# AITRICS/Medical_Tri_Modal_Pilot

Measured on AMD Instinct MI355X. Metric: tri-modal training samples/s (fwd+bwd+AdamW step, per-GPU batch 64), higher is better.
Workload: dtype bf16; 1 GPU; BASELINE configs[1]: vslt_img_txt tri_mbt_vsltcls, 6 layers, d_model 256, batch 64/GPU, TIE-len 1000 (N_v=1005), 224x224 CXR, 128-tok text, dropout 0.1, mbt-only-vslt 1, imgtxt-time 1; global_batch=64, parallelism=dp1

## Files before the change

include/mtmp.h:

```cpp
#ifndef MTMP_H
#define MTMP_H
#include <stdint.h>
#ifdef __cplusplus
extern "C" {
#endif

#define MTMP_F32 0
#define MTMP_BF16 1

int mtmp_abi_version(void);
const char* mtmp_last_error(void);

int mtmp_attn_fwd(int dtype, const void* q, const void* k, const void* v, void* o, const void* res, void* o_res,
                  float* lse, const int32_t* kv_len, const float* key_norms, int B, int N, int H, int ld_qkv, int ld_o,
                  float scale, void* stream);
int mtmp_attn_fwd_grouped(int dtype, int n, const void* const* q, const void* const* k, const void* const* v, void* const* o,
                          const void* const* res, void* const* o_res, float* const* lse, const int32_t* const* kv_len,
                          const int32_t* const* row_start, const float* const* key_norms, const int* N, const int* ld_qkv,
                          const int* ld_o, int B, int H, float scale, void* stream);
int mtmp_attn_bwd_grouped(int dtype, int n, const void* const* q, const void* const* k, const void* const* v,
                          const void* const* o, const void* const* d_o, const float* const* lse, const int32_t* const* kv_len,
                          const int32_t* const* row_start, void* const* dq, void* const* dk, void* const* dv,
                          float* const* delta_ws, const int* N, const int* ld_qkv, const int* ld_o, const int* ld_do,
                          const int* ld_dqkv, int B, int H, float scale, void* stream);
// ... 125 lines not shown
                             void* stream);
int mtmp_ln_gemm_signs_grouped(int dtype, int n, const void* const* x, const float* const* gamma, const float* const* beta,
                               const void* const* w, const float* const* bias, void* const* y, void* const* xn, float* const* stats,
                               void* const* signs, const int* M, int N, const int* ldx, float eps, float drop_p,
                               const unsigned* seeds, const unsigned* seed_dev, const int32_t* const* rows_live, void* stream);
int mtmp_gemm_nt_grouped(int dtype, int n, const void* const* a, const void* const* w, const float* const* bias,
                         const void* const* res, void* const* y, const int* M, int N, int K, const int* lda, const int* ldy,
                         const int* ldr, int act, float drop_p, const unsigned* seeds, const unsigned* seed_dev,
                         const int32_t* const* rows_live, void* stream);
int mtmp_gemm_nt_signs_drop_grouped(int dtype, int n, const void* const* a, const void* const* w, void* const* y, const int* M, int N,
                                    const int* lda, const void* const* signs, float gate_scale, float drop_p, const unsigned* seeds,
                                    const unsigned* seed_dev, void* const* a_out, const int32_t* const* rows_live, void* stream);
int mtmp_gemm_lnbwd_grouped(int dtype, int n, const void* const* dy, const void* const* wt, const void* const* z, const int* ldz,
                            const float* const* stats, const float* const* gamma, const void* const* d_res, const int* ldr,
                            void* const* dz, float* const* ws, const int* M, int K, const int* ldy, float eps,
                            const int32_t* const* rows_live, void* stream);
int mtmp_gemm_tn_group_plan(int n, const int* M, int N, int K, int* splits_out);
int mtmp_gemm_tn_grouped(int dtype, int n, const void* const* dy, const void* const* x, float* const* ws, const int* M, int N, int K,
                         const int* ldy, const int* ldx, const int* splits, const int32_t* const* rows_live, void* stream);

int mtmp_gemm_tn_slab_rows(int dtype, int M, int N, int K);
int mtmp_gemm_lnbwd_slab_rows(int M);
int mtmp_reduce_batch(const float* const* slab, const int* rows, const long long* cols, float* const* out_a, const long long* split,
                      float* const* out_b, int n, void* stream);

int mtmp_stream_input_slab_rows(int rows);
int mtmp_stream_input_bwd_partials(int dtype, const void* dz, const void* x, const float* cls, const float* gamma, const float* stats,
                                   void* dx, float* ws, int B, int N, int nb, float p, unsigned seed, const unsigned* seed_dev,
                                   const int32_t* row_start, const int32_t* kv_len, void* stream);
int mtmp_stream_input_bwd_grouped(int dtype, int n, const void* const* dz, const void* const* x, const float* const* cls,
                                  const float* const* gamma, const float* const* stats, void* const* dx, float* ws, const int* B,
                                  const int* N, const int* nb, const float* p, const unsigned* seed, const unsigned* seed_dev,
                                  const int32_t* const* row_start, const int32_t* const* kv_len, const void* const* add,
                                  const int* add_L, void* stream);
int mtmp_stream_input_fwd_add(int dtype, const void* x, const float* cls, const float* gamma, const float* beta, const float* pe,
                              const float* bott, void* out, float* stats, int B, int N, int nb, float eps, float p, unsigned seed,
                              const unsigned* seed_dev, const int32_t* row_start, const int32_t* kv_len, const void* add,
                              int add_L, void* stream);
int mtmp_token_sums(int dtype, int n, const void* const* dx, void* const* out, const int* rows, const int* L, void* stream);
int mtmp_tie_bwd_slab_rows(int n);
int mtmp_tie_time_embed_bwd_partials(int dtype, const float* events, int n, const float* time_events, int n_time, int n_time_a,
                                     const float* params, const void* d_out, const void* d_time_a, const void* d_time_b, float* ws,
                                     void* stream);
int mtmp_reduce_scatter(const float* const* src, const int* rows, const long long* ld, const long long* cols, float* const* out, int n,
                        void* stream);

int mtmp_publish_scalar(const float* value, unsigned* pair, void* stream);

int mtmp_copy_batch(const void* const* src, void* const* dst, const long long* bytes, const int* round16, int n, void* stream);

int mtmp_transpose_batch(int elem_bytes, const void* const* src, void* const* dst, const int* rows, const int* cols, int n,
                         void* stream);

int mtmp_stream_lengths(const long long* len_v, const long long* len_i, const long long* len_t, int* out, int B, int n_bott,
                        int txt_idx, void* stream);
int mtmp_image_slots(const long long* pattern, int present_below, int32_t* out, int B, int hw0, void* stream);
int mtmp_swin_stem_fwd_live(int dtype, const float* img, const float* w, const float* bias, const float* ln_w, const float* ln_b,
                            void* out, int n_img, int H, int W, const int32_t* order, const int32_t* rows_live, void* stream);
int mtmp_layernorm_rows_live(int dtype, const void* x, const float* w, const float* b, void* y, long long rows, int C, float eps,
                             int merge, int H, int W, const int32_t* rows_live, void* stream);
int mtmp_swin_ln_linear_live(int dtype, const void* x, const float* ln_w, const float* ln_b, const void* w, const float* bias,
                             void* y, long long M, int C, int N, float eps, const int32_t* rows_live, void* stream);
int mtmp_swin_mlp_live(int dtype, const void* x, const float* ln_w, const float* ln_b, const void* w1, const float* b1,
                       const void* w2, const float* b2, const float* row_scale, int rows_per_scale, void* y, long long M, int C,
                       float eps, const int32_t* rows_live, void* stream);
int mtmp_swin_window_attn_live(int dtype, const void* qkv, const void* table, void* out, int n_img, int H, int W, int C, int heads,
                               int shift, float scale, const int32_t* rows_live, void* stream);

int mtmp_layernorm_rows_bwd_slab_rows(long long rows, int C);
int mtmp_layernorm_rows_bwd(int dtype, const void* x, const float* w, const void* dy, void* dx, float* slab, long long rows, int C,
                            float eps, void* stream);
int mtmp_gelu_fwd(int dtype, const void* x, void* y, long long n, void* stream);
int mtmp_gelu_bwd(int dtype, const void* x, const void* dy, void* dx, long long n, void* stream);
int mtmp_swin_window_attn_bwd(int dtype, const void* qkv, const void* table, const void* dout, void* dqkv, float* dtab, int n_img,
                              int H, int W, int C, int heads, int shift, float scale, void* stream);

int mtmp_swin_attn_block(int dtype, const void* x, const float* ln_w, const float* ln_b, float eps, const void* wqkv,
                         const float* bqkv, const void* table, const void* wproj, const float* bproj, const float* row_scale,
                         void* out, int n_img, int H, int W, int C, int heads, int shift, float scale, const int32_t* rows_live,
                         void* stream);
int mtmp_gemm_nt_live(int dtype, const void* a, const void* w, const float* bias, const void* res, void* y, int M, int N, int K,
                      int lda, int ldy, int ldr, int act, float drop_p, unsigned seed, const unsigned* seed_dev, const void* gate,
                      float gate_scale, const float* row_scale, int rows_per_scale, const int32_t* rows_live, void* stream);

int mtmp_row_starts(const int32_t* kv_len, int32_t* out, int B, int n_max, void* stream);

#ifdef __cplusplus
}
#endif
#endif
```

medical_tri_modal_pilot_amd/_lib.py:

```python
import ctypes
import os
from ctypes import c_char_p, c_float, c_int, c_longlong, c_uint, c_void_p

_HERE = os.path.dirname(os.path.abspath(__file__))
LIB_PATH = os.environ.get("MTMP_LIB", os.path.join(_HERE, "libmtmp_hip.so"))

F32, BF16 = 0, 1

SIGNATURES = {
    "mtmp_abi_version": (c_int, []),
    "mtmp_last_error": (c_char_p, []),
    "mtmp_attn_fwd": (c_int, [c_int] + [c_void_p] * 9 + [c_int] * 5 + [c_float, c_void_p]),
    "mtmp_attn_cls_fwd": (c_int, [c_int] + [c_void_p] * 3 + [c_int, c_void_p, c_int] + [c_void_p] * 5 + [c_int] * 4 + [c_float, c_void_p]),
    "mtmp_attn_cls_bwd": (c_int, [c_int] + [c_void_p] * 3 + [c_int] + [c_void_p] * 8 + [c_int] * 5 + [c_float, c_void_p]),
    "mtmp_attn_fwd_grouped": (c_int, [c_int, c_int] + [c_void_p] * 13 + [c_int, c_int, c_float, c_void_p]),
    "mtmp_attn_bwd_grouped": (c_int, [c_int, c_int] + [c_void_p] * 17 + [c_int, c_int, c_float, c_void_p]),
    "mtmp_key_norms_floats": (c_longlong, [c_longlong, c_int]),
    "mtmp_key_norms": (c_int, [c_int, c_void_p, c_void_p, c_longlong, c_int, c_int, c_void_p]),
    "mtmp_attn_bwd": (c_int, [c_int] + [c_void_p] * 11 + [c_int] * 7 + [c_float, c_void_p]),
    "mtmp_ln_gemm": (c_int, [c_int] + [c_void_p] * 8 + [c_int] * 4 + [c_float, c_int, c_float, c_uint, c_void_p, c_void_p]),
    "mtmp_ln_gemm_qkv": (c_int, [c_int] + [c_void_p] * 9 + [c_int, c_int, c_float, c_void_p]),
    "mtmp_gemm_nt": (c_int, [c_int] + [c_void_p] * 5 + [c_int] * 7 + [c_float, c_uint, c_void_p, c_void_p, c_float, c_void_p, c_int,
                             c_void_p]),
    "mtmp_gemm_nt_live": (c_int, [c_int] + [c_void_p] * 5 + [c_int] * 7 + [c_float, c_uint, c_void_p, c_void_p, c_float, c_void_p, c_int,
                             c_void_p, c_void_p]),
    "mtmp_sign_bits_bytes": (c_longlong, [c_int, c_int]),
    "mtmp_ln_gemm_signs": (c_int, [c_int] + [c_void_p] * 8 + [c_int] * 4 + [c_float, c_float, c_uint, c_void_p, c_void_p, c_void_p]),
    "mtmp_gemm_nt_signs": (c_int, [c_int] + [c_void_p] * 3 + [c_int] * 4 + [c_void_p, c_float, c_void_p]),
    "mtmp_gemm_nt_signs_drop": (c_int, [c_int] + [c_void_p] * 3 + [c_int] * 4 + [c_void_p, c_float, c_float, c_uint, c_void_p,
                                                                                   c_void_p, c_void_p]),
    "mtmp_ln_gemm_qkv_grouped": (c_int, [c_int, c_int] + [c_void_p] * 11 + [c_float, c_void_p, c_void_p]),
    "mtmp_ln_gemm_signs_grouped": (c_int, [c_int, c_int] + [c_void_p] * 10 + [c_int, c_void_p, c_float, c_float, c_void_p, c_void_p,
                                                                                   c_void_p, c_void_p]),
    "mtmp_gemm_nt_grouped": (c_int, [c_int, c_int] + [c_void_p] * 6 + [c_int, c_int] + [c_void_p] * 3 + [c_int, c_float, c_void_p,
                                                                                                       c_void_p, c_void_p, c_void_p]),
    "mtmp_gemm_nt_signs_drop_grouped": (c_int, [c_int, c_int] + [c_void_p] * 4 + [c_int, c_void_p, c_void_p, c_float, c_float,
                                                                                  c_void_p, c_void_p, c_void_p, c_void_p, c_void_p]),
    "mtmp_gemm_lnbwd_grouped": (c_int, [c_int, c_int] + [c_void_p] * 11 + [c_int, c_void_p, c_float, c_void_p, c_void_p]),
    "mtmp_gemm_tn_group_plan": (c_int, [c_int, c_void_p, c_int, c_int, c_void_p]),
    "mtmp_gemm_tn_grouped": (c_int, [c_int, c_int] + [c_void_p] * 4 + [c_int, c_int] + [c_void_p] * 4 + [c_void_p]),
    "mtmp_gemm_tn_slab_rows": (c_int, [c_int] * 4),
    "mtmp_gemm_lnbwd_slab_rows": (c_int, [c_int]),
    "mtmp_reduce_batch": (c_int, [c_void_p] * 6 + [c_int, c_void_p]),
    "mtmp_reduce_scatter": (c_int, [c_void_p] * 5 + [c_int, c_void_p]),
    "mtmp_stream_input_slab_rows": (c_int, [c_int]),
    "mtmp_stream_input_bwd_partials": (c_int, [c_int] + [c_void_p] * 7 + [c_int] * 3 + [c_float, c_uint, c_void_p, c_void_p, c_void_p, c_void_p]),
    "mtmp_stream_input_bwd_grouped": (c_int, [c_int, c_int] + [c_void_p] * 18),
    "mtmp_stream_input_fwd_add": (c_int, [c_int] + [c_void_p] * 8 + [c_int] * 3 + [c_float, c_float, c_uint, c_void_p, c_void_p, c_void_p, c_void_p, c_int, c_void_p]),
    "mtmp_token_sums": (c_int, [c_int, c_int] + [c_void_p] * 5),
    "mtmp_tie_bwd_slab_rows": (c_int, [c_int]),
    "mtmp_tie_time_embed_bwd_partials": (c_int, [c_int, c_void_p, c_int, c_void_p, c_int, c_int] + [c_void_p] * 6),
    "mtmp_publish_scalar": (c_int, [c_void_p, c_void_p, c_void_p]),
    "mtmp_copy_batch": (c_int, [c_void_p] * 4 + [c_int, c_void_p]),
    "mtmp_stream_lengths": (c_int, [c_void_p] * 4 + [c_int] * 3 + [c_void_p]),
    "mtmp_row_starts": (c_int, [c_void_p, c_void_p, c_int, c_int, c_void_p]),
    "mtmp_image_slots": (c_int, [c_void_p, c_int, c_void_p, c_int, c_int, c_void_p]),
    "mtmp_transpose_batch": (c_int, [c_int, c_void_p, c_void_p, c_void_p, c_void_p, c_int, c_void_p]),
    "mtmp_layernorm_rows": (c_int, [c_int] + [c_void_p] * 4 + [c_longlong, c_int, c_float, c_int, c_int, c_int, c_void_p]),
    "mtmp_layernorm_rows_live": (c_int, [c_int] + [c_void_p] * 4 + [c_longlong, c_int, c_float, c_int, c_int, c_int, c_void_p, c_void_p]),
    "mtmp_swin_window_attn": (c_int, [c_int] + [c_void_p] * 3 + [c_int] * 6 + [c_float, c_void_p]),
    "mtmp_swin_window_attn_live": (c_int, [c_int] + [c_void_p] * 3 + [c_int] * 6 + [c_float, c_void_p, c_void_p]),
    "mtmp_layernorm_rows_bwd_slab_rows": (c_int, [c_longlong, c_int]),
    "mtmp_layernorm_rows_bwd": (c_int, [c_int] + [c_void_p] * 5 + [c_longlong, c_int, c_float, c_void_p]),
    "mtmp_gelu_fwd": (c_int, [c_int, c_void_p, c_void_p, c_longlong, c_void_p]),
    "mtmp_gelu_bwd": (c_int, [c_int, c_void_p, c_void_p, c_void_p, c_longlong, c_void_p]),
    "mtmp_swin_window_attn_bwd": (c_int, [c_int] + [c_void_p] * 5 + [c_int] * 6 + [c_float, c_void_p]),
    "mtmp_gemm_tn_ws_floats": (c_longlong, [c_int, c_int, c_int]),
    "mtmp_gemm_tn": (c_int, [c_int] + [c_void_p] * 5 + [c_int] * 5 + [c_void_p]),
    "mtmp_gemm_tn_live": (c_int, [c_int] + [c_void_p] * 5 + [c_int] * 5 + [c_void_p, c_void_p]),
    "mtmp_ln_bwd_ws_floats": (c_int, [c_int]),
    "mtmp_ln_bwd": (c_int, [c_int, c_void_p, c_int, c_void_p, c_void_p, c_void_p, c_void_p, c_int, c_void_p,
                            c_void_p, c_void_p, c_int, c_float, c_void_p]),
    "mtmp_gemm_lnbwd_ws_floats": (c_int, [c_int]),
    "mtmp_gemm_lnbwd": (c_int, [c_int, c_void_p, c_void_p, c_void_p, c_int, c_void_p, c_void_p, c_void_p, c_int, c_void_p,
                                c_void_p, c_void_p, c_int, c_int, c_int, c_float, c_void_p]),
    "mtmp_tie_embed_fwd": (c_int, [c_int] + [c_void_p] * 4 + [c_int, c_void_p]),
    "mtmp_tie_bwd_ws_floats": (c_int, [c_int]),
    "mtmp_tie_embed_bwd": (c_int, [c_int] + [c_void_p] * 5 + [c_int, c_void_p]),
    "mtmp_time_embed_fwd": (c_int, [c_int] + [c_void_p] * 4 + [c_int, c_void_p]),
    "mtmp_time_embed_bwd": (c_int, [c_int] + [c_void_p] * 5 + [c_int, c_void_p]),
    "mtmp_tie_embed_packed_fwd": (c_int, [c_int, c_void_p, c_void_p, c_int, c_int, c_void_p, c_void_p, c_void_p, c_void_p]),
    "mtmp_tie_embed_packed_bwd": (c_int, [c_int, c_void_p, c_void_p, c_int, c_int, c_void_p, c_void_p, c_void_p, c_void_p, c_void_p]),
    "mtmp_stream_input_ws_floats": (c_int, [c_int]),
    "mtmp_stream_input_fwd": (c_int, [c_int] + [c_void_p] * 8 + [c_int] * 3 + [c_float, c_float, c_uint, c_void_p, c_void_p, c_void_p, c_void_p]),
    "mtmp_stream_input_bwd": (c_int, [c_int] + [c_void_p] * 8 + [c_int] * 3 + [c_float, c_uint, c_void_p, c_void_p, c_void_p, c_void_p]),
    "mtmp_head_ws_floats": (c_int, [c_int]),
    "mtmp_head_fwd": (c_int, [c_void_p] * 6 + [c_int, c_float, c_float, c_float, c_int, c_void_p]),
    "mtmp_head_bwd": (c_int, [c_void_p] * 12 + [c_int, c_float, c_int, c_void_p]),
    "mtmp_head_fwd_t": (c_int, [c_int] + [c_void_p] * 6 + [c_int, c_float, c_float, c_float, c_int, c_void_p, c_void_p]),
    "mtmp_head_bwd_scatter": (c_int, [c_int] + [c_void_p] * 9 + [c_int, c_float, c_int, c_void_p]),
    "mtmp_bce_logits_mean": (c_int, [c_void_p] * 4 + [c_int, c_void_p]),
    "mtmp_timestamp": (c_int, [c_void_p, c_void_p]),
    "mtmp_swin_ln_linear": (c_int, [c_int] + [c_void_p] * 6 + [c_longlong, c_int, c_int, c_float, c_void_p]),
    "mtmp_swin_ln_linear_live": (c_int, [c_int] + [c_void_p] * 6 + [c_longlong, c_int, c_int, c_float, c_void_p, c_void_p]),
    "mtmp_swin_mlp": (c_int, [c_int] + [c_void_p] * 8 + [c_int, c_void_p, c_longlong, c_int, c_float, c_void_p]),
    "mtmp_swin_mlp_live": (c_int, [c_int] + [c_void_p] * 8 + [c_int, c_void_p, c_longlong, c_int, c_float, c_void_p, c_void_p]),
    "mtmp_swin_attn_block": (c_int, [c_int] + [c_void_p] * 3 + [c_float] + [c_void_p] * 7 + [c_int] * 6 + [c_float, c_void_p, c_void_p]),
    "mtmp_swin_stem_fwd": (c_int, [c_int] + [c_void_p] * 6 + [c_int] * 3 + [c_void_p]),
    "mtmp_swin_stem_fwd_live": (c_int, [c_int] + [c_void_p] * 6 + [c_int] * 3 + [c_void_p, c_void_p, c_void_p]),
    "mtmp_adamw_step": (c_int, [c_void_p] * 5 + [c_longlong] + [c_float] * 5 + [c_int, c_float, c_void_p]),
    "mtmp_bottleneck_exchange_fwd": (c_int, [c_int] + [c_void_p] * 3 + [c_int] * 4 + [c_void_p, c_int, c_void_p, c_void_p, c_void_p, c_void_p]),
    "mtmp_bottleneck_exchange_bwd": (c_int, [c_int] + [c_void_p] * 3 + [c_int] * 4 + [c_void_p, c_int, c_void_p, c_void_p, c_void_p, c_void_p]),
    "mtmp_dropout_bwd": (c_int, [c_int, c_void_p, c_void_p, c_longlong, c_uint, c_void_p, c_float, c_void_p]),
}

_lib = None


# ... 24 lines not shown
```

medical_tri_modal_pilot_amd/csrc/gemm.hip:

```cpp
#include "common.hip.h"
#include <type_traits>
template <int N> using template_int = std::integral_constant<int, N>;

namespace {

constexpr int BM = 128, BN = 128, BK = 64, LDW = BK + 8;

template <typename T> struct GemmArgs {
    const T* a; const T* w; const float* bias; const T* res; T* y;
    const float* gamma; const float* beta; T* xn; float* stats;
    int M, N, K, lda, ldy, ldr;
    float eps;
    float drop_p;
    unsigned seed;
    const unsigned* seed_dev;
    const T* gate;
    float gate_scale;
    int act;
    const float* row_scale;
    int rows_per_scale;
    unsigned short* signs = nullptr;
    float* knorm = nullptr;
    const int* m_live = nullptr;
};
// ... 1149 lines not shown
        g.seg[i] = segs[i < n ? i : 0];
        g.first[i] = total;
        if (i < n) total += blocks_of(segs[i]);
    }
    g.first[GRP_MAX] = total;
    return g;
}

int launch_ln_gemm_dma(int n, const GemmArgs<bf16>* segs, int relu, int gate, hipStream_t st) {
    using P = PanelDma;
    const GemmArgs<bf16>& a = segs[0];
    const bool drop = a.drop_p > 0.f, signs = !gate && relu && a.signs;
    for (int i = 1; i < n; ++i)
        if (segs[i].N != a.N || (segs[i].drop_p > 0.f) != drop || !segs[i].signs != !a.signs || !segs[i].knorm != !a.knorm ||
            !segs[i].gamma != !a.gamma) {
            mtmp_set_error("mtmp_ln_gemm (grouped): the streams of one launch must agree in N, dropout, sign bits and key norms");
            return MTMP_ERR_ARG;
        }
    const void* fs[7] = {(const void*)ln_gemm_dma_kernel<false, false, false, false>, (const void*)ln_gemm_dma_kernel<false, true, false, false>,
                         (const void*)ln_gemm_dma_kernel<true, false, false, false>, (const void*)ln_gemm_dma_kernel<true, true, false, false>,
                         (const void*)ln_gemm_dma_kernel<true, false, false, true>, (const void*)ln_gemm_dma_kernel<true, true, false, true>,
                         (const void*)ln_gemm_dma_kernel<false, false, true, false>};
    const bool knorm = a.knorm != nullptr;
    const int which = gate ? 6 : signs ? 4 + (drop ? 1 : 0) : (relu ? 2 : 0) + (drop ? 1 : 0);
    const void* fk = (const void*)ln_gemm_dma_kernel<false, false, false, false, true>;
    if (hipFuncSetAttribute(knorm ? fk : fs[which], hipFuncAttributeMaxDynamicSharedMemorySize, (int)P::lds_bytes) != hipSuccess) {
        mtmp_set_error("mtmp_ln_gemm: cannot raise dynamic LDS to %zu", P::lds_bytes);
        return MTMP_ERR_LAUNCH;
    }
    int mtiles;
    const Grouped<GemmArgs<bf16>> g = make_group(n, segs, [](const GemmArgs<bf16>& x) { return (x.M + BM - 1) / BM; }, mtiles);
    const int npanels = a.N / P::NP;
    int nsplit = 512 / mtiles;
    nsplit = nsplit < 1 ? 1 : (nsplit > npanels ? npanels : nsplit);
    const int need = (npanels + P::MAXP - 1) / P::MAXP;
    if (nsplit < need) nsplit = need;
    dim3 grid(mtiles, nsplit);
    if (knorm) {
        hipLaunchKernelGGL((ln_gemm_dma_kernel<false, false, false, false, true>), grid, dim3(256), P::lds_bytes, st, g);
        MTMP_CHECK_LAUNCH("mtmp_ln_gemm_qkv");
        return MTMP_OK;
    }
    switch (which) {
    case 0: hipLaunchKernelGGL((ln_gemm_dma_kernel<false, false, false, false>), grid, dim3(256), P::lds_bytes, st, g); break;
    case 1: hipLaunchKernelGGL((ln_gemm_dma_kernel<false, true, false, false>), grid, dim3(256), P::lds_bytes, st, g); break;
    case 2: hipLaunchKernelGGL((ln_gemm_dma_kernel<true, false, false, false>), grid, dim3(256), P::lds_bytes, st, g); break;
    case 3: hipLaunchKernelGGL((ln_gemm_dma_kernel<true, true, false, false>), grid, dim3(256), P::lds_bytes, st, g); break;
    case 4: hipLaunchKernelGGL((ln_gemm_dma_kernel<true, false, false, true>), grid, dim3(256), P::lds_bytes, st, g); break;
    case 5: hipLaunchKernelGGL((ln_gemm_dma_kernel<true, true, false, true>), grid, dim3(256), P::lds_bytes, st, g); break;
    default: hipLaunchKernelGGL((ln_gemm_dma_kernel<false, false, true, false>), grid, dim3(256), P::lds_bytes, st, g); break;
    }
    MTMP_CHECK_LAUNCH("mtmp_ln_gemm");
    return MTMP_OK;
}
template <typename T>
int launch_ln_gemm(GemmArgs<T> a, int relu, hipStream_t st) {
    const size_t sm = Panel<T>::lds_bytes;
    if (a.N % Panel<T>::NP != 0) {
        mtmp_set_error("mtmp_ln_gemm: N=%d must be a multiple of %d for this dtype", a.N, Panel<T>::NP);
        return MTMP_ERR_ARG;
    }
    if constexpr (sizeof(T) == 2) return launch_ln_gemm_dma(1, &a, relu, 0, st);
    if (sm > 48 * 1024) {
        const void* fs[4] = {(const void*)ln_gemm_kernel<T, false, false>, (const void*)ln_gemm_kernel<T, false, true>,
                             (const void*)ln_gemm_kernel<T, true, false>, (const void*)ln_gemm_kernel<T, true, true>};
        const void* f = fs[(relu ? 2 : 0) + (a.drop_p > 0.f ? 1 : 0)];
        if (hipFuncSetAttribute(f, hipFuncAttributeMaxDynamicSharedMemorySize, (int)sm) != hipSuccess) {
            mtmp_set_error("mtmp_ln_gemm: cannot raise dynamic LDS to %zu", sm);
            return MTMP_ERR_LAUNCH;
        }
    }
    const int mtiles = (a.M + BM - 1) / BM, npanels = a.N / Panel<T>::NP;
    int nsplit = 512 / mtiles;
    nsplit = nsplit < 1 ? 1 : (nsplit > npanels ? npanels : nsplit);
    dim3 grid(mtiles, nsplit);
    const bool drop = a.drop_p > 0.f;
    if (relu && drop)       hipLaunchKernelGGL((ln_gemm_kernel<T, true, true>), grid, dim3(256), sm, st, a);
    else if (relu)          hipLaunchKernelGGL((ln_gemm_kernel<T, true, false>), grid, dim3(256), sm, st, a);
    else if (drop)          hipLaunchKernelGGL((ln_gemm_kernel<T, false, true>), grid, dim3(256), sm, st, a);
    else                    hipLaunchKernelGGL((ln_gemm_kernel<T, false, false>), grid, dim3(256), sm, st, a);
    MTMP_CHECK_LAUNCH("mtmp_ln_gemm");
    return MTMP_OK;
}
template <typename T, int TM>
int launch_gemm_nt_tm(int n, const GemmArgs<T>* segs, int relu, hipStream_t st) {
    const GemmArgs<T>& a = segs[0];
    size_t sm = (size_t)(TM + BN) * LDW * sizeof(T);
    const size_t stage = (size_t)TM * LDO * sizeof(T);
    if (sm < stage) sm = stage;
    if (sm > 48 * 1024) {
        const void* fs[4] = {(const void*)gemm_nt_kernel<T, false, TM, false>, (const void*)gemm_nt_kernel<T, false, TM, true>,
                             (const void*)gemm_nt_kernel<T, true, TM, false>, (const void*)gemm_nt_kernel<T, true, TM, true>};
        const void* f = fs[(relu ? 2 : 0) + (a.drop_p > 0.f ? 1 : 0)];
        if (hipFuncSetAttribute(f, hipFuncAttributeMaxDynamicSharedMemorySize, (int)sm) != hipSuccess) {
            mtmp_set_error("mtmp_gemm_nt: cannot raise dynamic LDS to %zu", sm);
            return MTMP_ERR_LAUNCH;
        }
    }
    int nwg;
    const Grouped<GemmArgs<T>> g = make_group(n, segs, [](const GemmArgs<T>& x) { return ((x.M + TM - 1) / TM) * ((x.N + BN - 1) / BN); }, nwg);
    dim3 grid(nwg);
    const bool drop = a.drop_p > 0.f;
    if (relu && drop)       hipLaunchKernelGGL((gemm_nt_kernel<T, true, TM, true>), grid, dim3(256), sm, st, g);
    else if (relu)          hipLaunchKernelGGL((gemm_nt_kernel<T, true, TM, false>), grid, dim3(256), sm, st, g);
    else if (drop)          hipLaunchKernelGGL((gemm_nt_kernel<T, false, TM, true>), grid, dim3(256), sm, st, g);
    else                    hipLaunchKernelGGL((gemm_nt_kernel<T, false, TM, false>), grid, dim3(256), sm, st, g);
    MTMP_CHECK_LAUNCH("mtmp_gemm_nt");
    return MTMP_OK;
}
template <typename T>
int launch_gemm_nt(int n, const GemmArgs<T>* segs, int relu, hipStream_t st) {
    long long wgs128 = 0;
    for (int i = 0; i < n; ++i) {
        wgs128 += (long long)((segs[i].M + 127) / 128) * ((segs[i].N + BN - 1) / BN);
        if (segs[i].N != segs[0].N || segs[i].K != segs[0].K || segs[i].act != segs[0].act ||
            (segs[i].drop_p > 0.f) != (segs[0].drop_p > 0.f)) {
            mtmp_set_error("mtmp_gemm_nt (grouped): the streams of one launch must agree in N, K, activation and dropout");
            return MTMP_ERR_ARG;
        }
    }
    return wgs128 < 512 ? launch_gemm_nt_tm<T, 64>(n, segs, relu, st) : launch_gemm_nt_tm<T, 128>(n, segs, relu, st);
}
constexpr int LDXT = 256 + 8;

template <typename T> struct LnBwdGemmArgs {
    const T* dy; const T* wt; const T* z; const float* stats; const float* gamma; const T* d_res; T* dz; float* slab;
    int M, K, ldy, ldz, ldr;
    float eps;
    const int* m_live = nullptr;
};

template <typename T>
__global__ __launch_bounds__(256, (sizeof(T) == 2 ? 2 : 1)) void gemm_lnbwd_kernel(Grouped<LnBwdGemmArgs<T>> grp) {
    extern __shared__ __attribute__((aligned(16))) char smem_raw[];
    const int seg = grp_find(grp, (int)blockIdx.x);
    const LnBwdGemmArgs<T>& p = grp.seg[seg];
    const int bx = (int)blockIdx.x - grp.first[seg];
    T* sA = reinterpret_cast<T*>(smem_raw);
    T* sW = sA + 128 * LDW;
    const int tid = threadIdx.x, lane = tid & 63, wave = tid >> 6, r = lane & 31, half = lane >> 5;
    const int wr = wave & 1, wc = wave >> 1;
    const int m0 = bx * 128;
    const int nk = (p.K + BK - 1) / BK;
    const int M = live_rows(p.M, p.m_live);
    if (m0 >= M) {
        for (int i = tid; i < 512; i += 256) p.slab[(size_t)bx * 512 + i] = 0.f;
        return;
    }
    TileRegs<T> areg, wreg0, wreg1;
    tile_fetch<T>(areg, p.dy, p.ldy, m0, M, 0, tid, p.K);
    tile_fetch<T>(wreg0, p.wt, p.K, 0, 256, 0, tid, p.K);
    tile_fetch<T>(wreg1, p.wt, p.K, 128, 256, 0, tid, p.K);
    f32x16 acc[2][4];
#pragma unroll
    for (int rt = 0; rt < 2; ++rt)
#pragma unroll
        for (int nt = 0; nt < 4; ++nt) acc[rt][nt] = f32x16{0};
    for (int kc = 0; kc < nk; ++kc) {
        __syncthreads();
        tile_commit<T>(sA, areg, tid);
        tile_commit<T>(sW, wreg0, tid);
        tile_commit<T>(sW + 128 * LDW, wreg1, tid);
        __syncthreads();
        if (kc + 1 < nk) {
            tile_fetch<T>(areg, p.dy, p.ldy, m0, M, (kc + 1) * BK, tid, p.K);
            tile_fetch<T>(wreg0, p.wt, p.K, 0, 256, (kc + 1) * BK, tid, p.K);
            tile_fetch<T>(wreg1, p.wt, p.K, 128, 256, (kc + 1) * BK, tid, p.K);
        }
#pragma unroll
        for (int c = 0; c < 4; ++c) {
            Frag<T> a[2];
#pragma unroll
            for (int rt = 0; rt < 2; ++rt) a[rt] = frag_load<T>(sA + (64 * wr + 32 * rt + r) * LDW + 16 * c + 8 * half);
#pragma unroll
            for (int nt = 0; nt < 4; ++nt) {
                const Frag<T> w = frag_load<T>(sW + (128 * wc + 32 * nt + r) * LDW + 16 * c + 8 * half);
#pragma unroll
                for (int rt = 0; rt < 2; ++rt) mma<T>(acc[rt][nt], w, a[rt]);
            }
        }
    }
    __syncthreads();
    T* sX = reinterpret_cast<T*>(smem_raw);
#pragma unroll
    for (int rt = 0; rt < 2; ++rt)
#pragma unroll
        for (int nt = 0; nt < 4; ++nt)
#pragma unroll
            for (int g = 0; g < 4; ++g)
                store4<T>(sX + (64 * wr + 32 * rt + r) * LDXT + 128 * wc + 32 * nt + 8 * g + 4 * half, acc[rt][nt][4 * g],
                          acc[rt][nt][4 * g + 1], acc[rt][nt][4 * g + 2], acc[rt][nt][4 * g + 3]);
    __syncthreads();
    const f32x4 gm = ld4f(p.gamma + 4 * lane);
    float part[2][4] = {{0.f, 0.f, 0.f, 0.f}, {0.f, 0.f, 0.f, 0.f}};
// ... 160 lines not shown
static int ln_gemm_entry(int dtype, const void* x, const float* gamma, const float* beta, const void* w, const float* bias,
                         void* y, void* xn, float* stats, int M, int N, int ldx, int ldy, float eps, int relu, float drop_p,
                         unsigned seed, const unsigned* seed_dev, void* signs, void* stream) {
    MTMP_CHECK_ARG(x && gamma && beta && w && y, "mtmp_ln_gemm: null pointer");
    MTMP_CHECK_ARG(M > 0 && N > 0 && N % 32 == 0 && ldx >= 256 && ldx % 8 == 0 && ldy >= N && ldy % 8 == 0,
                   "mtmp_ln_gemm: bad shape M=%d N=%d ldx=%d ldy=%d (K is fixed at 256)", M, N, ldx, ldy);
    MTMP_CHECK_ARG(drop_p >= 0.f && drop_p < 1.f && (double)M * N < 4294967296.0, "mtmp_ln_gemm: bad dropout %f", drop_p);
    MTMP_CHECK_ARG(!signs || (dtype == 1 && relu && N % PanelDma::NP == 0), "mtmp_ln_gemm_signs: bf16, ReLU and N %% 64 == 0 only");
    hipStream_t st = (hipStream_t)stream;
    if (dtype == 0) {
        GemmArgs<float> a{(const float*)x, (const float*)w, bias, nullptr, (float*)y, gamma, beta, (float*)xn, stats,
                          M, N, 256, ldx, ldy, 0, eps, drop_p, seed, seed_dev, nullptr, 1.f, 0, nullptr, 1};
        return launch_ln_gemm<float>(a, relu, st);
    }
    if (dtype == 1) {
        GemmArgs<bf16> a{(const bf16*)x, (const bf16*)w, bias, nullptr, (bf16*)y, gamma, beta, (bf16*)xn, stats,
                         M, N, 256, ldx, ldy, 0, eps, drop_p, seed, seed_dev, nullptr, 1.f, 0, nullptr, 1, (unsigned short*)signs};
        return launch_ln_gemm<bf16>(a, relu, st);
    }
    mtmp_set_error("mtmp_ln_gemm: unknown dtype %d", dtype);
    return MTMP_ERR_ARG;
}
extern "C" int mtmp_ln_gemm(int dtype, const void* x, const float* gamma, const float* beta, const void* w,
                            const float* bias, void* y, void* xn, float* stats, int M, int N, int ldx, int ldy,
                            float eps, int relu, float drop_p, unsigned seed, const unsigned* seed_dev, void* stream) {
    return ln_gemm_entry(dtype, x, gamma, beta, w, bias, y, xn, stats, M, N, ldx, ldy, eps, relu, drop_p, seed, seed_dev, nullptr, stream);
}
extern "C" int mtmp_key_norms(int dtype, const void* k, float* out, long long rows, int H, int ld, void* stream);
extern "C" int mtmp_ln_gemm_qkv(int dtype, const void* x, const float* gamma, const float* beta, const void* w, const float* bias,
                                void* y, void* xn, float* stats, float* key_norms, int M, int ldx, float eps, void* stream) {
    MTMP_CHECK_ARG(x && gamma && beta && w && y && key_norms, "mtmp_ln_gemm_qkv: null pointer");
    MTMP_CHECK_ARG(M > 0 && ldx >= 256 && ldx % 8 == 0, "mtmp_ln_gemm_qkv: bad shape M=%d ldx=%d", M, ldx);
    if (dtype == 1) {
        GemmArgs<bf16> a{(const bf16*)x, (const bf16*)w, bias, nullptr, (bf16*)y, gamma, beta, (bf16*)xn, stats,
                         M, 768, 256, ldx, 768, 0, eps, 0.f, 0u, nullptr, nullptr, 1.f, 0, nullptr, 1, nullptr, key_norms};
        return launch_ln_gemm_dma(1, &a, 0, 0, (hipStream_t)stream);
    }
    if (int e = ln_gemm_entry(dtype, x, gamma, beta, w, bias, y, xn, stats, M, 768, ldx, 768, eps, 0, 0.f, 0u, nullptr, nullptr, stream)) return e;
    const size_t es = dtype == 0 ? 4 : 2;
    return mtmp_key_norms(dtype, (const char*)y + 256 * es, key_norms, M, 4, 768, stream);
}
extern "C" long long mtmp_sign_bits_bytes(int M, int N) { return (long long)(N / 32) * M * 4; }
extern "C" int mtmp_ln_gemm_signs(int dtype, const void* x, const float* gamma, const float* beta, const void* w,
                                  const float* bias, void* y, void* xn, float* stats, int M, int N, int ldx, int ldy,
                                  float eps, float drop_p, unsigned seed, const unsigned* seed_dev, void* signs, void* stream) {
    MTMP_CHECK_ARG(signs, "mtmp_ln_gemm_signs: null pointer");
    return ln_gemm_entry(dtype, x, gamma, beta, w, bias, y, xn, stats, M, N, ldx, ldy, eps, 1, drop_p, seed, seed_dev, signs, stream);
}
extern "C" int mtmp_gemm_nt_signs(int dtype, const void* a, const void* w, void* y, int M, int N, int lda, int ldy,
                                  const void* signs, float gate_scale, void* stream) {
    MTMP_CHECK_ARG(a && w && y && signs, "mtmp_gemm_nt_signs: null pointer");
    MTMP_CHECK_ARG(dtype == 1, "mtmp_gemm_nt_signs: bf16 only (dtype %d)", dtype);
    MTMP_CHECK_ARG(M > 0 && N > 0 && N % PanelDma::NP == 0 && lda >= 256 && lda % 8 == 0 && ldy >= N && ldy % 8 == 0,
                   "mtmp_gemm_nt_signs: bad shape M=%d N=%d lda=%d ldy=%d (K is fixed at 256)", M, N, lda, ldy);
    GemmArgs<bf16> g{(const bf16*)a, (const bf16*)w, nullptr, nullptr, (bf16*)y, nullptr, nullptr, nullptr, nullptr, M, N, 256, lda, ldy,
                     0, 0.f, 0.f, 0u, nullptr, nullptr, gate_scale, 0, nullptr, 1, (unsigned short*)signs};
    return launch_ln_gemm_dma(1, &g, 0, 1, (hipStream_t)stream);
}

extern "C" int mtmp_gemm_nt_signs_drop(int dtype, const void* a, const void* w, void* y, int M, int N, int lda, int ldy,
                                       const void* signs, float gate_scale, float drop_p, unsigned seed, const unsigned* seed_dev,
                                       void* a_out, void* stream) {
    MTMP_CHECK_ARG(a && w && y && signs, "mtmp_gemm_nt_signs_drop: null pointer");
    MTMP_CHECK_ARG(dtype == 1, "mtmp_gemm_nt_signs_drop: bf16 only (dtype %d)", dtype);
    MTMP_CHECK_ARG(M > 0 && M < (1 << 24) && N > 0 && N % PanelDma::NP == 0 && lda >= 256 && lda % 8 == 0 && ldy >= N && ldy % 8 == 0 &&
                       drop_p >= 0.f && drop_p < 1.f,
                   "mtmp_gemm_nt_signs_drop: bad argument M=%d N=%d lda=%d ldy=%d p=%f (K is fixed at 256)", M, N, lda, ldy, drop_p);
    GemmArgs<bf16> g{(const bf16*)a, (const bf16*)w, nullptr, nullptr, (bf16*)y, nullptr, nullptr, (bf16*)a_out, nullptr, M, N, 256, lda,
                     ldy, 0, 0.f, drop_p, seed, seed_dev, nullptr, gate_scale, 0, nullptr, 1, (unsigned short*)signs};
    return launch_ln_gemm_dma(1, &g, 0, 1, (hipStream_t)stream);
}

extern "C" int mtmp_gemm_nt_live(int dtype, const void* a, const void* w, const float* bias, const void* res, void* y,
                                 int M, int N, int K, int lda, int ldy, int ldr, int act, float drop_p, unsigned seed,
                                 const unsigned* seed_dev, const void* gate, float gate_scale, const float* row_scale,
                                 int rows_per_scale, const int32_t* rows_live, void* stream);
extern "C" int mtmp_gemm_nt(int dtype, const void* a, const void* w, const float* bias, const void* res, void* y,
                            int M, int N, int K, int lda, int ldy, int ldr, int act, float drop_p, unsigned seed,
                            const unsigned* seed_dev, const void* gate, float gate_scale, const float* row_scale,
                            int rows_per_scale, void* stream) {
    return mtmp_gemm_nt_live(dtype, a, w, bias, res, y, M, N, K, lda, ldy, ldr, act, drop_p, seed, seed_dev, gate, gate_scale,
                             row_scale, rows_per_scale, nullptr, stream);
}
extern "C" int mtmp_gemm_nt_live(int dtype, const void* a, const void* w, const float* bias, const void* res, void* y,
                                 int M, int N, int K, int lda, int ldy, int ldr, int act, float drop_p, unsigned seed,
                                 const unsigned* seed_dev, const void* gate, float gate_scale, const float* row_scale,
                                 int rows_per_scale, const int32_t* rows_live, void* stream) {
    MTMP_CHECK_ARG(a && w && y, "mtmp_gemm_nt: null pointer");
    MTMP_CHECK_ARG(M > 0 && N > 0 && K > 0 && K % 8 == 0 && N % 32 == 0 && lda >= K && lda % 8 == 0 && ldy >= N &&
                       ldy % 8 == 0 && (!res || (ldr >= N && ldr % 8 == 0)),
                   "mtmp_gemm_nt: bad shape M=%d N=%d K=%d lda=%d ldy=%d ldr=%d", M, N, K, lda, ldy, ldr);
    MTMP_CHECK_ARG(drop_p >= 0.f && drop_p < 1.f && (double)M * N < 4294967296.0, "mtmp_gemm_nt: bad dropout %f", drop_p);
    MTMP_CHECK_ARG(act >= 0 && act <= 2 && (!row_scale || rows_per_scale > 0), "mtmp_gemm_nt: bad act %d / row_scale", act);
    hipStream_t st = (hipStream_t)stream;
    if (dtype == 0) {
        GemmArgs<float> g{(const float*)a, (const float*)w, bias, (const float*)res, (float*)y, nullptr, nullptr,
                          nullptr, nullptr, M, N, K, lda, ldy, ldr, 0.f, drop_p, seed, seed_dev, (const float*)gate, gate_scale, act, row_scale,
                          rows_per_scale};
        g.m_live = rows_live;
        return launch_gemm_nt<float>(1, &g, 0, st);
    }
    if (dtype == 1) {
        GemmArgs<bf16> g{(const bf16*)a, (const bf16*)w, bias, (const bf16*)res, (bf16*)y, nullptr, nullptr, nullptr,
                         nullptr, M, N, K, lda, ldy, ldr, 0.f, drop_p, seed, seed_dev, (const bf16*)gate, gate_scale, act, row_scale,
                         rows_per_scale};
        g.m_live = rows_live;
        return launch_gemm_nt<bf16>(1, &g, 0, st);
    }
    mtmp_set_error("mtmp_gemm_nt: unknown dtype %d", dtype);
    return MTMP_ERR_ARG;
}

extern "C" int mtmp_gemm_lnbwd_ws_floats(int M) { return ((M + 127) / 128 + RED_GROUPS) * 512; }

extern "C" int mtmp_gemm_lnbwd(int dtype, const void* dy, const void* wt, const void* z, int ldz, const float* stats,
                               const float* gamma, const void* d_res, int ldr, void* dz, float* dgamma_dbeta, float* ws,
                               int M, int K, int ldy, float eps, void* stream) {
    MTMP_CHECK_ARG(dy && wt && z && stats && gamma && dz && ws, "mtmp_gemm_lnbwd: null pointer");
    MTMP_CHECK_ARG(M > 0 && K > 0 && K % 8 == 0 && ldy >= K && ldy % 8 == 0 && ldz >= 256 && ldz % 4 == 0 &&
                       (!d_res || (ldr >= 256 && ldr % 4 == 0)), "mtmp_gemm_lnbwd: bad shape M=%d K=%d ldy=%d ldz=%d", M, K, ldy, ldz);
    hipStream_t st = (hipStream_t)stream;
    if (dtype == 0) {
        LnBwdGemmArgs<float> a{(const float*)dy, (const float*)wt, (const float*)z, stats, gamma, (const float*)d_res,
                               (float*)dz, nullptr, M, K, ldy, ldz, ldr, eps};
        return launch_gemm_lnbwd<float>(1, &a, &dgamma_dbeta, &ws, st);
    }
    if (dtype == 1) {
        LnBwdGemmArgs<bf16> a{(const bf16*)dy, (const bf16*)wt, (const bf16*)z, stats, gamma, (const bf16*)d_res,
                              (bf16*)dz, nullptr, M, K, ldy, ldz, ldr, eps};
        return launch_gemm_lnbwd<bf16>(1, &a, &dgamma_dbeta, &ws, st);
    }
    mtmp_set_error("mtmp_gemm_lnbwd: unknown dtype %d", dtype);
    return MTMP_ERR_ARG;
}

extern "C" int mtmp_gemm_tn_slab_rows(int dtype, int M, int N, int K) { return tn_launch_splits(dtype == 1, M, N, K, nullptr); }
extern "C" int mtmp_gemm_lnbwd_slab_rows(int M) { return (M + 127) / 128; }
namespace {
int launch_reduce_batch(const float* const* slab, const int* rows, const long long* cols, const long long* ld, float* const* out_a,
                        const long long* split, float* const* out_b, int n, hipStream_t st, const char* who) {
    ReduceBatch t;
    long long most = 0;
    for (int i = 0; i < RB_MAX; ++i) {
        const int k = i < n ? i : 0;
        const long long ldk = ld ? ld[k] : cols[k];
        MTMP_CHECK_ARG(slab[k] && out_a[k] && rows[k] > 0 && cols[k] > 0 && split[k] >= 0 && split[k] <= cols[k] && ldk >= cols[k],
                       "%s: bad entry %d", who, k);
        t.slab[i] = slab[k]; t.a[i] = out_a[k]; t.b[i] = out_b ? out_b[k] : nullptr; t.cols[i] = cols[k]; t.split[i] = split[k];
        t.rows[i] = rows[k]; t.ld[i] = ldk;
        most = most > cols[k] ? most : cols[k];
    }
    long long blocks = (most + 255) / 256;
    for (int i = 0; i < n; ++i) {
        const int rl = rows[i] >= 256 ? 64 : rows[i] >= 64 ? 16 : 4;
        const long long need = (cols[i] + 4 * (256 / rl) - 1) / (4 * (256 / rl));
        blocks = blocks > need ? blocks : need;
    }
    hipLaunchKernelGGL(reduce_batch_kernel, dim3((unsigned)(blocks > 4096 ? 4096 : blocks), n), dim3(256), 0, st, t);
    MTMP_CHECK_LAUNCH(who);
    return MTMP_OK;
}
}
extern "C" int mtmp_reduce_batch(const float* const* slab, const int* rows, const long long* cols, float* const* out_a,
                                 const long long* split, float* const* out_b, int n, void* stream) {
    MTMP_CHECK_ARG(slab && rows && cols && out_a && split && out_b && n > 0 && n <= RB_MAX, "mtmp_reduce_batch: bad argument (n=%d)", n);
    return launch_reduce_batch(slab, rows, cols, nullptr, out_a, split, out_b, n, (hipStream_t)stream, "mtmp_reduce_batch");
}
extern "C" int mtmp_reduce_scatter(const float* const* src, const int* rows, const long long* ld, const long long* cols,
                                   float* const* out, int n, void* stream) {
    MTMP_CHECK_ARG(src && rows && ld && cols && out && n > 0 && n <= RB_MAX, "mtmp_reduce_scatter: bad argument (n=%d)", n);
    return launch_reduce_batch(src, rows, cols, ld, out, cols, nullptr, n, (hipStream_t)stream, "mtmp_reduce_scatter");
}

extern "C" long long mtmp_gemm_tn_ws_floats(int M, int N, int K) {
    return (long long)tn_splits(M, N, K, 640) * ((long long)N * K + N);
}

extern "C" int mtmp_gemm_tn_live(int dtype, const void* dy, const void* x, float* dw, float* db, float* ws, int M, int N,
                                 int K, int ldy, int ldx, const int32_t* rows_live, void* stream);
extern "C" int mtmp_gemm_tn(int dtype, const void* dy, const void* x, float* dw, float* db, float* ws, int M, int N,
                            int K, int ldy, int ldx, void* stream) {
    return mtmp_gemm_tn_live(dtype, dy, x, dw, db, ws, M, N, K, ldy, ldx, nullptr, stream);
}
extern "C" int mtmp_gemm_tn_live(int dtype, const void* dy, const void* x, float* dw, float* db, float* ws, int M, int N,
                                 int K, int ldy, int ldx, const int32_t* rows_live, void* stream) {
    MTMP_CHECK_ARG(dy && x && ws && (dw || !db), "mtmp_gemm_tn: null pointer");
    MTMP_CHECK_ARG(M > 0 && N > 0 && K > 0 && N % 128 == 0 && K % 128 == 0 && ldy >= N && ldx >= K && ldy % 8 == 0 &&
                       ldx % 8 == 0, "mtmp_gemm_tn: bad shape M=%d N=%d K=%d ldy=%d ldx=%d", M, N, K, ldy, ldx);
    hipStream_t st = (hipStream_t)stream;
    if (dtype == 0) return launch_gemm_tn<float>(dy, x, dw, db, ws, M, N, K, ldy, ldx, rows_live, st);
// ... 159 lines not shown
```

Before: 8488 samples/s.

## Add wide-tile bf16 GEMM core with auto-selection for large single-stream GEMMs

Adds a new bf16 GEMM kernel with 128- or 256-row tiles, a multi-stage async LDS ring and an LDS-staged epilogue. launch_gemm_nt now routes large single-segment GEMMs (K>=256, >=1 GFLOP, no dropout or gate) to it automatically. Bigger tiles give more operand reuse per load and fewer workgroups. The cost is fewer workgroups for mid-sized shapes, higher LDS use per block and a new selection heuristic. It also exposes explicit core-choice entry points.

```diff
diff --git a/include/mtmp.h b/include/mtmp.h
--- a/include/mtmp.h
+++ b/include/mtmp.h
@@ -231,6 +231,11 @@
 int mtmp_gemm_nt_live(int dtype, const void* a, const void* w, const float* bias, const void* res, void* y, int M, int N, int K,
                       int lda, int ldy, int ldr, int act, float drop_p, unsigned seed, const unsigned* seed_dev, const void* gate,
                       float gate_scale, const float* row_scale, int rows_per_scale, const int32_t* rows_live, void* stream);
+int mtmp_gemm_nt_core(int core, int dtype, const void* a, const void* w, const float* bias, const void* res, void* y, int M, int N,
+                      int K, int lda, int ldy, int ldr, int act, float drop_p, unsigned seed, const unsigned* seed_dev,
+                      const void* gate, float gate_scale, const float* row_scale, int rows_per_scale, const int32_t* rows_live,
+                      void* stream);
+int mtmp_gemm_nt_core_pick(int dtype, int n_streams, int M, int N, int K, int lda, int act, float drop_p, int gated);
 
 int mtmp_row_starts(const int32_t* kv_len, int32_t* out, int B, int n_max, void* stream);
 
diff --git a/medical_tri_modal_pilot_amd/_lib.py b/medical_tri_modal_pilot_amd/_lib.py
--- a/medical_tri_modal_pilot_amd/_lib.py
+++ b/medical_tri_modal_pilot_amd/_lib.py
@@ -24,6 +24,9 @@
                              c_void_p]),
     "mtmp_gemm_nt_live": (c_int, [c_int] + [c_void_p] * 5 + [c_int] * 7 + [c_float, c_uint, c_void_p, c_void_p, c_float, c_void_p, c_int,
                              c_void_p, c_void_p]),
+    "mtmp_gemm_nt_core": (c_int, [c_int, c_int] + [c_void_p] * 5 + [c_int] * 7 + [c_float, c_uint, c_void_p, c_void_p, c_float, c_void_p,
+                                                                                  c_int, c_void_p, c_void_p]),
+    "mtmp_gemm_nt_core_pick": (c_int, [c_int] * 7 + [c_float, c_int]),
     "mtmp_sign_bits_bytes": (c_longlong, [c_int, c_int]),
     "mtmp_ln_gemm_signs": (c_int, [c_int] + [c_void_p] * 8 + [c_int] * 4 + [c_float, c_float, c_uint, c_void_p, c_void_p, c_void_p]),
     "mtmp_gemm_nt_signs": (c_int, [c_int] + [c_void_p] * 3 + [c_int] * 4 + [c_void_p, c_float, c_void_p]),
diff --git a/medical_tri_modal_pilot_amd/csrc/gemm.hip b/medical_tri_modal_pilot_amd/csrc/gemm.hip
--- a/medical_tri_modal_pilot_amd/csrc/gemm.hip
+++ b/medical_tri_modal_pilot_amd/csrc/gemm.hip
@@ -1255,6 +1255,168 @@
     MTMP_CHECK_LAUNCH("mtmp_ln_gemm");
     return MTMP_OK;
 }
+
+template <int TM> struct WideGeom {
+    static constexpr int NW = TM / 32, THREADS = 64 * NW;
+    static constexpr int NS = TM == 256 ? 3 : 4;
+    static constexpr int ROWB = BK * 2;
+    static constexpr int A_BYTES = TM * ROWB, STAGE = A_BYTES + BN * ROWB;
+    static constexpr int APW = 4, WPW = BN / 8 / NW, DPW = APW + WPW;
+    static constexpr size_t ring_bytes = (size_t)NS * STAGE, out_bytes = (size_t)TM * LDO * 2;
+    static constexpr size_t lds_bytes = ring_bytes > out_bytes ? ring_bytes : out_bytes;
+    static_assert(lds_bytes <= 160 * 1024 && APW * 8 * NW == TM && WPW * 8 * NW == BN, "wide core geometry");
+};
+
+template <int TM>
+__global__ __launch_bounds__(WideGeom<TM>::THREADS, 1) void gemm_nt_wide_kernel(GemmArgs<bf16> p) {
+    using T = bf16;
+    using G = WideGeom<TM>;
+    const int ntn = p.N / BN;
+    const int M = live_rows(p.M, p.m_live);
+    int wg = xcd_remap(blockIdx.x, gridDim.x);
+    if (p.m_live) {
+        const int live = ((M + TM - 1) / TM) * ntn;
+        if ((int)blockIdx.x >= live) return;
+        wg = xcd_remap(blockIdx.x, live);
+    }
+    const int m0 = (wg / ntn) * TM, n0 = (wg % ntn) * BN;
+    if (m0 >= M) return;
+    extern __shared__ __attribute__((aligned(16))) char smem_raw[];
+    const unsigned lds0 = (unsigned)(uintptr_t)((__attribute__((address_space(3))) char*)smem_raw);
+    const int tid = threadIdx.x, lane = tid & 63, wave = __builtin_amdgcn_readfirstlane(tid >> 6), r = lane & 31, half = lane >> 5;
+    const int nk = p.K / BK;
+    const unsigned ldab = (unsigned)p.lda * 2u, ldwb = (unsigned)p.K * 2u;
+    unsigned aoff[G::APW], woff[G::WPW];
+#pragma unroll
+    for (int i = 0; i < G::APW; ++i) {
+        const int row = 32 * wave + 8 * i + (lane >> 3);
+        aoff[i] = (unsigned)min(m0 + row, M - 1) * ldab + 16u * (unsigned)((lane & 7) ^ ((row >> 1) & 7));
+    }
+#pragma unroll
+    for (int i = 0; i < G::WPW; ++i) {
+        const int row = 8 * (G::WPW * wave + i) + (lane >> 3);
+        woff[i] = (unsigned)(n0 + row) * ldwb + 16u * (unsigned)((lane & 7) ^ ((row >> 1) & 7));
+    }
+    auto issue = [&](int s) __attribute__((always_inline)) {
+        const unsigned buf = lds0 + (unsigned)((s % G::NS) * G::STAGE);
+        const char* asrc = reinterpret_cast<const char*>(p.a) + (size_t)s * G::ROWB;
+        const char* wsrc = reinterpret_cast<const char*>(p.w) + (size_t)s * G::ROWB;
+#pragma unroll
+        for (int i = 0; i < G::APW; ++i) dma16(aoff[i], asrc, buf + (unsigned)(G::APW * wave + i) * 1024u);
+#pragma unroll
+        for (int i = 0; i < G::WPW; ++i) dma16(woff[i], wsrc, buf + (unsigned)G::A_BYTES + (unsigned)(G::WPW * wave + i) * 1024u);
+    };
+    int roff[4];
+#pragma unroll
+    for (int c = 0; c < 4; ++c) roff[c] = r * G::ROWB + 16 * ((2 * c + half) ^ ((r >> 1) & 7));
+    f32x16 acc[4];
+#pragma unroll
+    for (int nt = 0; nt < 4; ++nt) acc[nt] = f32x16{0};
+#pragma unroll
+    for (int s = 0; s < G::NS - 1; ++s)
+        if (s < nk) issue(s);
+    for (int s = 0; s < nk; ++s) {
+        tn_wait_stages<G::DPW>(min(nk - 1 - s, G::NS - 2));
+        __syncthreads();
+        if (s + G::NS - 1 < nk) issue(s + G::NS - 1);
+        const char* sa = smem_raw + (s % G::NS) * G::STAGE + 32 * wave * G::ROWB;
+        const char* sw = smem_raw + (s % G::NS) * G::STAGE + G::A_BYTES;
+        Frag<T> a[4], w[4][4];
+#pragma unroll
+        for (int c = 0; c < 4; ++c) {
+            a[c].v = *reinterpret_cast<const bf16x8*>(sa + roff[c]);
+#pragma unroll
+            for (int nt = 0; nt < 4; ++nt) w[c][nt].v = *reinterpret_cast<const bf16x8*>(sw + 32 * nt * G::ROWB + roff[c]);
+        }
+#pragma unroll
+        for (int c = 0; c < 4; ++c)
+#pragma unroll
+            for (int nt = 0; nt < 4; ++nt) mma<T>(acc[nt], w[c][nt], a[c]);
+    }
+    __syncthreads();
+    T* sOut = reinterpret_cast<T*>(smem_raw);
+    constexpr int PS = 8, RPP = G::THREADS / 16;
+    const int c8 = (tid & 15) * 8, gcol = n0 + c8;
+    Frag<T> rv[PS];
+    if (p.res) {
+#pragma unroll
+        for (int ps = 0; ps < PS; ++ps) rv[ps] = frag_load<T>(p.res + (size_t)min(m0 + (tid >> 4) + RPP * ps, M - 1) * p.ldr + gcol);
+    }
+    const int rl = 32 * wave + r;
+#pragma unroll
+    for (int nt = 0; nt < 4; ++nt) {
+#pragma unroll
+        for (int g = 0; g < 4; ++g) {
+            const int cl = 32 * nt + 8 * g + 4 * half;
+            f32x4 bv = {0.f, 0.f, 0.f, 0.f};
+            if (p.bias) bv = *reinterpret_cast<const f32x4*>(p.bias + n0 + cl);
+            float v[4];
+#pragma unroll
+            for (int i = 0; i < 4; ++i) v[i] = acc[nt][4 * g + i] + bv[i];
+            if (p.act == 1) {
+#pragma unroll
+                for (int i = 0; i < 4; ++i) v[i] = relu1(v[i]);
+            }
+            if (p.act == 2) {
+#pragma unroll
+                for (int i = 0; i < 4; ++i) v[i] = gelu<T>(v[i]);
+            }
+            store4<T>(sOut + rl * LDO + cl, v[0], v[1], v[2], v[3]);
+        }
+    }
+    __syncthreads();
+#pragma unroll
+    for (int ps = 0; ps < PS; ++ps) {
+        const int rl2 = (tid >> 4) + RPP * ps, grow = min(m0 + rl2, M - 1);
+        Frag<T> o = frag_load<T>(sOut + rl2 * LDO + c8);
+        if (p.row_scale || p.res) {
+            float v[8];
+#pragma unroll
+            for (int i = 0; i < 8; ++i) v[i] = to_f32(o.v[i]);
+            if (p.row_scale) {
+                const float rsv = p.row_scale[grow / p.rows_per_scale];
+#pragma unroll
+                for (int i = 0; i < 8; ++i) v[i] *= rsv;
+            }
+            if (p.res) {
+#pragma unroll
+                for (int i = 0; i < 8; ++i) v[i] = round_as<T>(v[i]) + to_f32(rv[ps].v[i]);
+            }
+#pragma unroll
+            for (int i = 0; i < 8; ++i) o.v[i] = from_f32<T>(v[i]);
+        }
+        frag_store<T>(p.y + (size_t)grow * p.ldy + gcol, o);
+    }
+}
+
+constexpr int CORE_ROW = 1, CORE_WIDE = 2, CORE_WIDE128 = 3, CORE_WIDE256 = 4;
+bool wide_ok(int n, const GemmArgs<bf16>* segs) {
+    const GemmArgs<bf16>& a = segs[0];
+    return n == 1 && a.drop_p == 0.f && !a.gate && a.K % BK == 0 && a.N % BN == 0 && a.lda % 8 == 0 &&
+           (double)a.M * a.lda * 2.0 < 2147483648.0 && (double)a.N * a.K * 2.0 < 2147483648.0;
+}
+int wide_rows(const GemmArgs<bf16>& a) {
+    const long long t128 = (long long)((a.M + 127) / 128) * (a.N / BN), t256 = (long long)((a.M + 255) / 256) * (a.N / BN);
+    return ((t256 + 255) / 256) * 256 <= ((t128 + 255) / 256) * 128 ? 256 : 128;
+}
+int gemm_nt_auto_core(int n, const GemmArgs<bf16>* segs) {
+    const GemmArgs<bf16>& a = segs[0];
+    if (!wide_ok(n, segs)) return CORE_ROW;
+    return a.K >= 256 && 2.0 * a.M * a.N * a.K >= 1073741824.0 ? CORE_WIDE : CORE_ROW;
+}
+template <int TM> int launch_gemm_nt_wide(const GemmArgs<bf16>& a, hipStream_t st) {
+    using G = WideGeom<TM>;
+    if (hipFuncSetAttribute((const void*)gemm_nt_wide_kernel<TM>, hipFuncAttributeMaxDynamicSharedMemorySize, (int)G::lds_bytes) !=
+        hipSuccess) {
+        mtmp_set_error("mtmp_gemm_nt: cannot raise dynamic LDS to %zu", G::lds_bytes);
+        return MTMP_ERR_LAUNCH;
+    }
+    const int tiles = ((a.M + TM - 1) / TM) * (a.N / BN);
+    hipLaunchKernelGGL(gemm_nt_wide_kernel<TM>, dim3(tiles), dim3(G::THREADS), G::lds_bytes, st, a);
+    MTMP_CHECK_LAUNCH("mtmp_gemm_nt (wide)");
+    return MTMP_OK;
+}
+
 template <typename T, int TM>
 int launch_gemm_nt_tm(int n, const GemmArgs<T>* segs, int relu, hipStream_t st) {
     const GemmArgs<T>& a = segs[0];
@@ -1282,7 +1444,21 @@
     return MTMP_OK;
 }
 template <typename T>
-int launch_gemm_nt(int n, const GemmArgs<T>* segs, int relu, hipStream_t st) {
+int launch_gemm_nt(int n, const GemmArgs<T>* segs, int relu, hipStream_t st, int core = 0) {
+    if constexpr (sizeof(T) == 2) {
+        if (core == 0 && !relu) core = gemm_nt_auto_core(n, segs);
+        if (core >= CORE_WIDE) {
+            if (relu || !wide_ok(n, segs)) {
+                mtmp_set_error("mtmp_gemm_nt: the wide core needs one bf16 stream, no dropout or gate, K %% 64 == 0 and N %% 128 == 0");
+                return MTMP_ERR_ARG;
+            }
+            const int tm = core == CORE_WIDE128 ? 128 : core == CORE_WIDE256 ? 256 : wide_rows(segs[0]);
+            return tm == 256 ? launch_gemm_nt_wide<256>(segs[0], st) : launch_gemm_nt_wide<128>(segs[0], st);
+        }
+    } else if (core >= CORE_WIDE) {
+        mtmp_set_error("mtmp_gemm_nt: the wide core is bf16 only");
+        return MTMP_ERR_ARG;
+    }
     long long wgs128 = 0;
     for (int i = 0; i < n; ++i) {
         wgs128 += (long long)((segs[i].M + 127) / 128) * ((segs[i].N + BN - 1) / BN);
@@ -1609,10 +1785,30 @@
     return mtmp_gemm_nt_live(dtype, a, w, bias, res, y, M, N, K, lda, ldy, ldr, act, drop_p, seed, seed_dev, gate, gate_scale,
                              row_scale, rows_per_scale, nullptr, stream);
 }
+extern "C" int mtmp_gemm_nt_core(int core, int dtype, const void* a, const void* w, const float* bias, const void* res, void* y,
+                                 int M, int N, int K, int lda, int ldy, int ldr, int act, float drop_p, unsigned seed,
+                                 const unsigned* seed_dev, const void* gate, float gate_scale, const float* row_scale,
+                                 int rows_per_scale, const int32_t* rows_live, void* stream);
 extern "C" int mtmp_gemm_nt_live(int dtype, const void* a, const void* w, const float* bias, const void* res, void* y,
                                  int M, int N, int K, int lda, int ldy, int ldr, int act, float drop_p, unsigned seed,
                                  const unsigned* seed_dev, const void* gate, float gate_scale, const float* row_scale,
                                  int rows_per_scale, const int32_t* rows_live, void* stream) {
+    return mtmp_gemm_nt_core(0, dtype, a, w, bias, res, y, M, N, K, lda, ldy, ldr, act, drop_p, seed, seed_dev, gate, gate_scale,
+                             row_scale, rows_per_scale, rows_live, stream);
+}
+extern "C" int mtmp_gemm_nt_core_pick(int dtype, int n_streams, int M, int N, int K, int lda, int act, float drop_p, int gated) {
+    if (dtype != 1 || n_streams != 1) return CORE_ROW;
+    static const bf16 gate_stub = (bf16)0.0f;
+    GemmArgs<bf16> g{};
+    g.M = M; g.N = N; g.K = K; g.lda = lda; g.act = act; g.drop_p = drop_p;
+    g.gate = gated ? &gate_stub : nullptr;
+    return gemm_nt_auto_core(1, &g);
+}
+extern "C" int mtmp_gemm_nt_core(int core, int dtype, const void* a, const void* w, const float* bias, const void* res, void* y,
+                                 int M, int N, int K, int lda, int ldy, int ldr, int act, float drop_p, unsigned seed,
+                                 const unsigned* seed_dev, const void* gate, float gate_scale, const float* row_scale,
+                                 int rows_per_scale, const int32_t* rows_live, void* stream) {
+    MTMP_CHECK_ARG(core >= 0 && core <= CORE_WIDE256, "mtmp_gemm_nt_core: unknown core %d", core);
     MTMP_CHECK_ARG(a && w && y, "mtmp_gemm_nt: null pointer");
     MTMP_CHECK_ARG(M > 0 && N > 0 && K > 0 && K % 8 == 0 && N % 32 == 0 && lda >= K && lda % 8 == 0 && ldy >= N &&
                        ldy % 8 == 0 && (!res || (ldr >= N && ldr % 8 == 0)),
@@ -1625,14 +1821,14 @@
                           nullptr, nullptr, M, N, K, lda, ldy, ldr, 0.f, drop_p, seed, seed_dev, (const float*)gate, gate_scale, act, row_scale,
                           rows_per_scale};
         g.m_live = rows_live;
-        return launch_gemm_nt<float>(1, &g, 0, st);
+        return launch_gemm_nt<float>(1, &g, 0, st, core);
     }
     if (dtype == 1) {
         GemmArgs<bf16> g{(const bf16*)a, (const bf16*)w, bias, (const bf16*)res, (bf16*)y, nullptr, nullptr, nullptr,
                          nullptr, M, N, K, lda, ldy, ldr, 0.f, drop_p, seed, seed_dev, (const bf16*)gate, gate_scale, act, row_scale,
                          rows_per_scale};
         g.m_live = rows_live;
-        return launch_gemm_nt<bf16>(1, &g, 0, st);
+        return launch_gemm_nt<bf16>(1, &g, 0, st, core);
     }
     mtmp_set_error("mtmp_gemm_nt: unknown dtype %d", dtype);
     return MTMP_ERR_ARG;
```

After: 8384 samples/s, median of 2. -1.2%, worse.
